# bayesiains/nflows

Measured on AMD Instinct MI355X. Metric: log_prob samples/sec (dim=64, K=8, 32-layer RQ-NSF) + max |fwd∘inv − x|, higher is better.
Workload: dtype f32 (inputs, outputs, spline arithmetic, accumulation; conditioner GEMMs: every fp32 operand carried as 3 f16 pieces = 33 significand bits, i.e. at the reference's own fp32 operand width, 5 cross products per multiply-add -- 3 on the f16 MFMA, the 2 at the 2^-22 level from the pieces' high bytes on

## Files before the change

### nflows_amd/csrc/f16x3_gemm.hpp

```cpp
#pragma once

#include "bf16x3_gemm.hpp"

namespace nfa {

typedef _Float16 f16x8 __attribute__((ext_vector_type(8)));
typedef int i32x8 __attribute__((ext_vector_type(8)));

namespace k8x {

constexpr int kScaleA = 119, kScaleB = 127;

#ifdef NFA_ABL_NO_MFMA
#define NFA_K8X_F16(a, b, c) (c)
#define NFA_K8X_BF8(a, b, c) (c)
#else
#define NFA_K8X_F16(a, b, c) __builtin_amdgcn_mfma_f32_32x32x16_f16(a, b, c, 0, 0, 0)
#define NFA_K8X_BF8(a, b, c) __builtin_amdgcn_mfma_scale_f32_32x32x64_f8f6f4(a, b, c, 1, 1, 0, kScaleA, 0, kScaleB)
#endif

struct Pieces {
    uvec4 h, l, r;
};

#define NFA_K8X_ASM asm volatile

__device__ __forceinline__ void split3_scaled(float v0, float v1, float scale, unsigned& hi, unsigned& lo, unsigned& rr) {
#if defined(NFA_K8X_NO_ASM)
    typedef _Float16 h2 __attribute__((ext_vector_type(2)));
    const float x0 = v0 * scale, x1 = v1 * scale;
    const h2 h = {(_Float16)x0, (_Float16)x1};
    const float t0 = x0 - (float)h[0], t1 = x1 - (float)h[1];
    const h2 l = {(_Float16)t0, (_Float16)t1};
    const h2 r = {(_Float16)((t0 - (float)l[0]) * 256.0f), (_Float16)((t1 - (float)l[1]) * 256.0f)};
    hi = __builtin_bit_cast(unsigned, h);
    lo = __builtin_bit_cast(unsigned, l);
    rr = __builtin_bit_cast(unsigned, r);
#else
    unsigned h, l, r;
    float t0, t1;
    NFA_K8X_ASM(
        "v_fma_mixlo_f16 %0, %5, %7, 0 op_sel_hi:[0,0,0]\n\t"
        "v_fma_mixhi_f16 %0, %6, %7, 0 op_sel_hi:[0,0,0]\n\t"
        "v_fma_mix_f32 %3, %5, %7, -%0 op_sel_hi:[0,0,1]\n\t"
        "v_fma_mix_f32 %4, %6, %7, -%0 op_sel:[0,0,1] op_sel_hi:[0,0,1]\n\t"
        "v_fma_mixlo_f16 %1, %3, 1.0, 0 op_sel_hi:[0,0,0]\n\t"
        "v_fma_mixhi_f16 %1, %4, 1.0, 0 op_sel_hi:[0,0,0]\n\t"
        "v_fma_mix_f32 %3, %3, 1.0, -%1 op_sel_hi:[0,0,1]\n\t"
        "v_fma_mix_f32 %4, %4, 1.0, -%1 op_sel:[0,0,1] op_sel_hi:[0,0,1]\n\t"
        "v_fma_mixlo_f16 %2, %3, %8, 0 op_sel_hi:[0,0,0]\n\t"
        "v_fma_mixhi_f16 %2, %4, %8, 0 op_sel_hi:[0,0,0]"
        : "=&v"(h), "=&v"(l), "=&v"(r), "=&v"(t0), "=&v"(t1)
        : "v"(v0), "v"(v1), "v"(scale), "s"(256.0f));
    hi = h;
    lo = l;
    rr = r;
#endif
}

__device__ __forceinline__ void pieces_fma2(unsigned h, unsigned l, unsigned r, float mul, float& acc0, float& acc1) {
    float t0, t1;
#if defined(NFA_K8X_NO_ASM)
    typedef _Float16 h2 __attribute__((ext_vector_type(2)));
    const h2 hh = __builtin_bit_cast(h2, h), ll = __builtin_bit_cast(h2, l), rr = __builtin_bit_cast(h2, r);
    t0 = ((float)hh[0] + (float)ll[0]) + (float)rr[0] * 0.00390625f;
    t1 = ((float)hh[1] + (float)ll[1]) + (float)rr[1] * 0.00390625f;
#else
    NFA_K8X_ASM(
        "v_fma_mix_f32 %0, %2, 1.0, %3 op_sel_hi:[1,0,1]\n\t"
        "v_fma_mix_f32 %1, %2, 1.0, %3 op_sel:[1,0,1] op_sel_hi:[1,0,1]\n\t"
        "v_fma_mix_f32 %0, %4, %5, %0 op_sel_hi:[1,0,0]\n\t"
        "v_fma_mix_f32 %1, %4, %5, %1 op_sel:[1,0,0] op_sel_hi:[1,0,0]"
        : "=&v"(t0), "=&v"(t1)
        : "v"(h), "v"(l), "v"(r), "s"(0.00390625f));
#endif
    acc0 = __builtin_fmaf(t0, mul, acc0);
    acc1 = __builtin_fmaf(t1, mul, acc1);
}

__device__ __forceinline__ void relu_pieces(Pieces& p) {
#pragma unroll
    for (int i = 0; i < 4; ++i) {
        unsigned keep;
        asm volatile("v_pk_min_i16 %0, %1, 0\n\t"
            "v_pk_add_i16 %0, %0, %2\n\t"
            "v_pk_ashrrev_i16 %0, %3, %0\n\t"
            "v_not_b32 %0, %0"
            : "=&v"(keep)
            : "v"(p.h[i]), "s"(0x03FF03FFu), "s"(0x000F000Fu));
        p.h[i] &= keep;
        p.l[i] &= keep;
        p.r[i] &= keep;
    }
}

__device__ __forceinline__ i32x8 bf8_operand(const Pieces& p0, const Pieces& p1) {
    constexpr unsigned kHigh = 0x07050301u;
    i32x8 b;
    b[0] = (int)__builtin_amdgcn_perm(p0.r[1], p0.r[0], kHigh);
    b[1] = (int)__builtin_amdgcn_perm(p0.r[3], p0.r[2], kHigh);
    b[2] = (int)__builtin_amdgcn_perm(p0.h[1], p0.h[0], kHigh);
    b[3] = (int)__builtin_amdgcn_perm(p0.h[3], p0.h[2], kHigh);
    b[4] = (int)__builtin_amdgcn_perm(p1.r[1], p1.r[0], kHigh);
    b[5] = (int)__builtin_amdgcn_perm(p1.r[3], p1.r[2], kHigh);
    b[6] = (int)__builtin_amdgcn_perm(p1.h[1], p1.h[0], kHigh);
    b[7] = (int)__builtin_amdgcn_perm(p1.h[3], p1.h[2], kHigh);
    return b;
}

template <bool RELU>
__device__ __forceinline__ void tile_to_pieces(const f32x16& a, float scale, Pieces& p0, Pieces& p1) {
    asm volatile("s_nop 7\n\ts_nop 3" : : "v"(a));
#pragma unroll
    for (int q2 = 0; q2 < 8; ++q2) {
        float v0 = a[q2 * 2], v1 = a[q2 * 2 + 1];
        if (RELU) {
            v0 = v0 < 0.0f ? 0.0f : v0;
            v1 = v1 < 0.0f ? 0.0f : v1;
        }
        unsigned h, l, r;
        split3_scaled(v0, v1, scale, h, l, r);
        if (q2 < 4) {
            p0.h[q2] = h;
            p0.l[q2] = l;
            p0.r[q2] = r;
        } else {
            p1.h[q2 - 4] = h;
            p1.l[q2 - 4] = l;
            p1.r[q2 - 4] = r;
        }
    }
}

__device__ __forceinline__ void add_pieces(f32x16& a, int q0, const Pieces& p, float mul) {
#pragma unroll
    for (int j2 = 0; j2 < 4; ++j2) {
        float a0 = a[q0 + 2 * j2], a1 = a[q0 + 2 * j2 + 1];
        pieces_fma2(p.h[j2], p.l[j2], p.r[j2], mul, a0, a1);
        a[q0 + 2 * j2] = a0;
        a[q0 + 2 * j2 + 1] = a1;
    }
}

__device__ __forceinline__ i32x8 join_x(vec4f lo, vec4f hi) {
    const uvec4 a = __builtin_bit_cast(uvec4, lo), b = __builtin_bit_cast(uvec4, hi);
    return i32x8{(int)a[0], (int)a[1], (int)a[2], (int)a[3], (int)b[0], (int)b[1], (int)b[2], (int)b[3]};
}

struct Lead {
    vec4f h0, l0, h1, l1;
};
__device__ __forceinline__ Lead read_lead(const vec4f* stage) {
    return Lead{stage[0 * 64], stage[1 * 64], stage[2 * 64], stage[3 * 64]};
}

#define NFA_K8X_FENCE() __builtin_amdgcn_sched_barrier(0)

template <bool LAST>
__device__ __forceinline__ void stage_kmajor(f32x16& acc0, f32x16& acc1, const Pieces& b0, const Pieces& b1, const i32x8& bx,
                                             WeightStream& sm, int lane, Lead& lead) {
    stream_request(sm);
    const vec4f* cur = sm.ring + sm.slot * kStageVec4 + lane;
    const f16x8 bh0 = __builtin_bit_cast(f16x8, b0.h), bl0 = __builtin_bit_cast(f16x8, b0.l);
    const f16x8 bh1 = __builtin_bit_cast(f16x8, b1.h), bl1 = __builtin_bit_cast(f16x8, b1.l);
    const vec4f x0l = cur[4 * 64], x0h = cur[5 * 64];
    const vec4f h0 = cur[6 * 64], l0 = cur[7 * 64], h1 = cur[8 * 64], l1 = cur[9 * 64], x1l = cur[10 * 64], x1h = cur[11 * 64];
    NFA_K8X_FENCE();
    {
        const f16x8 ah0 = __builtin_bit_cast(f16x8, lead.h0), al0 = __builtin_bit_cast(f16x8, lead.l0);
        const f16x8 ah1 = __builtin_bit_cast(f16x8, lead.h1), al1 = __builtin_bit_cast(f16x8, lead.l1);
        acc0 = NFA_K8X_F16(ah0, bl0, acc0);
        acc0 = NFA_K8X_F16(al0, bh0, acc0);
        acc0 = NFA_K8X_F16(ah0, bh0, acc0);
        acc0 = NFA_K8X_F16(ah1, bl1, acc0);
        acc0 = NFA_K8X_F16(al1, bh1, acc0);
        acc0 = NFA_K8X_F16(ah1, bh1, acc0);
        acc0 = NFA_K8X_BF8(join_x(x0l, x0h), bx, acc0);
    }
    const f16x8 ah0 = __builtin_bit_cast(f16x8, h0), al0 = __builtin_bit_cast(f16x8, l0);
    const f16x8 ah1 = __builtin_bit_cast(f16x8, h1), al1 = __builtin_bit_cast(f16x8, l1);
    const i32x8 ax = join_x(x1l, x1h);
    acc1 = NFA_K8X_F16(ah0, bl0, acc1);
    acc1 = NFA_K8X_F16(al0, bh0, acc1);
    acc1 = NFA_K8X_F16(ah0, bh0, acc1);
    NFA_K8X_FENCE();
    stream_advance(sm);
    if constexpr (!LAST) lead = read_lead(sm.ring + sm.slot * kStageVec4 + lane);
    NFA_K8X_FENCE();
    acc1 = NFA_K8X_F16(ah1, bl1, acc1);
    acc1 = NFA_K8X_F16(al1, bh1, acc1);
    acc1 = NFA_K8X_F16(ah1, bh1, acc1);
    acc1 = NFA_K8X_BF8(ax, bx, acc1);
}

template <bool RELU, int NKS>
__device__ __forceinline__ void gemm_kmajor(f32x16 (&acc)[4], const Pieces (&p)[8], WeightStream& sm, int lane) {
    static_assert(NKS % 2 == 0, "pairs of k-steps");
    Lead lead = read_lead(sm.ring + sm.slot * kStageVec4 + lane);
#pragma unroll
    for (int pr = 0; pr < NKS / 2; ++pr) {
        Pieces b0 = p[2 * pr], b1 = p[2 * pr + 1];
        if (RELU) {
            relu_pieces(b0);
            relu_pieces(b1);
        }
        const i32x8 bx = bf8_operand(b0, b1);
        stage_kmajor<false>(acc[0], acc[1], b0, b1, bx, sm, lane, lead);
        if (pr + 1 < NKS / 2) stage_kmajor<false>(acc[2], acc[3], b0, b1, bx, sm, lane, lead);
        else stage_kmajor<true>(acc[2], acc[3], b0, b1, bx, sm, lane, lead);
    }
}

}
}
```

### nflows_amd/csrc/rqs_resnet_f16x3_kernel.hpp

```cpp
#pragma once

#include "f16x3_gemm.hpp"
#include "rqs_resnet_f16_kernel.hpp"

#include <hip/hip_ext.h>
#include <stdlib.h>

namespace nfa {
namespace k8x {

struct Args {
    const float* x;
    const vec4f* w;
    const float* bias;
    const float* scales;
    const int32_t* tables;
    float* out;
    float* lad;
    int32_t* redo;
    int32_t* status;
    int64_t batch;
    int D, dt, di, num_blocks, num_layers, num_stages, bias_per_layer, accumulate;
    RqsDev sp;
    int normal, skip_out;
    float log_z, act_scale;
    int Ds;
    float* dbg_logits;
};

typedef __attribute__((address_space(3))) float lds_f32;

using nfa::load_bias_tile;

__device__ __forceinline__ void load_bias_tile(f32x16& acc, const lds_f32* bias_tile_half) {
    typedef __attribute__((address_space(3))) const vec4f lds_vec4f;
    lds_vec4f* bp = reinterpret_cast<lds_vec4f*>(bias_tile_half);
#pragma unroll
    for (int q4 = 0; q4 < 4; ++q4) {
        const vec4f b = bp[q4];
        acc[q4 * 4 + 0] = b.x;
        acc[q4 * 4 + 1] = b.y;
        acc[q4 * 4 + 2] = b.z;
        acc[q4 * 4 + 3] = b.w;
    }
}

template <int N>
__device__ __forceinline__ void uniform_load(const float* p, float (&v)[N]) {
    static_assert(N == 2 || N == 4, "one or two pairs");
    uint64_t v01, v23 = 0;
    if constexpr (N == 2)
        asm volatile("s_load_dwordx2 %0, %1, 0x0\n\ts_waitcnt lgkmcnt(0)" : "=&s"(v01) : "s"(p) : "memory");
    else
        asm volatile("s_load_dwordx2 %0, %2, 0x0\n\ts_load_dwordx2 %1, %2, 0x8\n\ts_waitcnt lgkmcnt(0)"
                     : "=&s"(v01), "=&s"(v23) : "s"(p) : "memory");
    v[0] = __builtin_bit_cast(float, (unsigned)v01);
    v[1] = __builtin_bit_cast(float, (unsigned)(v01 >> 32));
    if constexpr (N == 4) {
        v[2] = __builtin_bit_cast(float, (unsigned)v23);
        v[3] = __builtin_bit_cast(float, (unsigned)(v23 >> 32));
    }
}

struct NoWeave {
    template <int U0, int U1>
    __device__ __forceinline__ void span() {}
};
template <int UNIT, class Steps>
struct UnitWeave {
    Steps &fa, &fb;
    const RqsDev& sp;
    template <int U0, int U1>
    __device__ __forceinline__ void span() {
        constexpr int N = k8h::spline_unit_slices<UNIT, Steps>();
        k8h::spline_unit_range<UNIT, (U0 * N) / 32, (U1 * N) / 32>(fa, fb, sp);
    }
};
template <int MASK, class Steps>
struct SeqWeave {
    Steps& f;
    const RqsDev& sp;
    template <int U0, int U1>
    __device__ __forceinline__ void span() {
        constexpr int N = k8h::spline_seq_count<MASK, Steps>();
        k8h::spline_seq_range<MASK, (U0 * N) / 32, (U1 * N) / 32>(f, sp);
    }
};

#define NFA_K8X_PUMP_F16(U, A_, B_)                                         \
    acc = NFA_K8X_F16(A_, B_, acc);                                         \
    __builtin_amdgcn_sched_barrier(0);                                      \
    w.template span<(U), (U) + 1>();                                        \
    __builtin_amdgcn_sched_barrier(0)
#define NFA_K8X_PUMP_BF8(U, A_, B_)                                         \
    acc = NFA_K8X_BF8(A_, B_, acc);                                         \
    __builtin_amdgcn_sched_barrier(0);                                      \
    w.template span<(U), (U) + 2>();                                        \
    __builtin_amdgcn_sched_barrier(0)

template <int HS, class W>
__device__ __forceinline__ void stage_pumped(f32x16& acc, const Pieces (&p)[8], const i32x8 (&bx)[4], WeightStream& sm, int lane,
                                             Lead& lead, W& w) {
    stream_request(sm);
    const vec4f* cur = sm.ring + sm.slot * kStageVec4 + lane;
    vec4f xa = cur[8 * 64], xb = cur[9 * 64];
    vec4f fh0 = lead.h0, fl0 = lead.l0, fh1 = lead.h1, fl1 = lead.l1;
    {
        const Pieces& b0 = p[HS * 4 + 0];
        const Pieces& b1 = p[HS * 4 + 1];
        const f16x8 bh0 = __builtin_bit_cast(f16x8, b0.h), bl0 = __builtin_bit_cast(f16x8, b0.l);
        const f16x8 bh1 = __builtin_bit_cast(f16x8, b1.h), bl1 = __builtin_bit_cast(f16x8, b1.l);
        const f16x8 ah0 = __builtin_bit_cast(f16x8, fh0), al0 = __builtin_bit_cast(f16x8, fl0);
        const f16x8 ah1 = __builtin_bit_cast(f16x8, fh1), al1 = __builtin_bit_cast(f16x8, fl1);
        const i32x8 ax = join_x(xa, xb);
        NFA_K8X_PUMP_F16(HS * 16 + 0, ah0, bl0);
        NFA_K8X_PUMP_F16(HS * 16 + 1, al0, bh0);
        NFA_K8X_PUMP_F16(HS * 16 + 2, ah0, bh0);
        fh0 = cur[4 * 64];
        fl0 = cur[5 * 64];
        NFA_K8X_PUMP_F16(HS * 16 + 3, ah1, bl1);
        NFA_K8X_PUMP_F16(HS * 16 + 4, al1, bh1);
        NFA_K8X_PUMP_F16(HS * 16 + 5, ah1, bh1);
        fh1 = cur[6 * 64];
        fl1 = cur[7 * 64];
        NFA_K8X_PUMP_BF8(HS * 16 + 6, ax, bx[HS * 2 + 0]);
        xa = cur[10 * 64];
        xb = cur[11 * 64];
    }
    {
        const Pieces& b0 = p[HS * 4 + 2];
        const Pieces& b1 = p[HS * 4 + 3];
        const f16x8 bh0 = __builtin_bit_cast(f16x8, b0.h), bl0 = __builtin_bit_cast(f16x8, b0.l);
        const f16x8 bh1 = __builtin_bit_cast(f16x8, b1.h), bl1 = __builtin_bit_cast(f16x8, b1.l);
        const f16x8 ah0 = __builtin_bit_cast(f16x8, fh0), al0 = __builtin_bit_cast(f16x8, fl0);
        const f16x8 ah1 = __builtin_bit_cast(f16x8, fh1), al1 = __builtin_bit_cast(f16x8, fl1);
        const i32x8 ax = join_x(xa, xb);
        NFA_K8X_PUMP_F16(HS * 16 + 8, ah0, bl0);
        NFA_K8X_PUMP_F16(HS * 16 + 9, al0, bh0);
        NFA_K8X_PUMP_F16(HS * 16 + 10, ah0, bh0);
        NFA_K8X_PUMP_F16(HS * 16 + 11, ah1, bl1);
        NFA_K8X_PUMP_F16(HS * 16 + 12, al1, bh1);
        NFA_K8X_PUMP_F16(HS * 16 + 13, ah1, bh1);
        stream_advance(sm);
        lead = read_lead(sm.ring + sm.slot * kStageVec4 + lane);
        __builtin_amdgcn_sched_barrier(0);
        NFA_K8X_PUMP_BF8(HS * 16 + 14, ax, bx[HS * 2 + 1]);
    }
}
#undef NFA_K8X_PUMP_F16
#undef NFA_K8X_PUMP_BF8

template <class W>
__device__ __forceinline__ void gemm_tile_pumped(f32x16& acc, const Pieces (&p)[8], const i32x8 (&bx)[4], WeightStream& sm, int lane,
                                                 Lead& lead, W&& w) {
    stage_pumped<0>(acc, p, bx, sm, lane, lead, w);
    stage_pumped<1>(acc, p, bx, sm, lane, lead, w);
}

template <int TI, int T, int KB, class Steps, class BiasPtr>
__device__ __forceinline__ void any_group_tiles(f32x16& acc, Steps& f, BiasPtr gb, const Pieces (&p)[8], const i32x8 (&bx)[4],
                                                WeightStream& sm, int lane, Lead& lead, const RqsDev& sp) {
    if constexpr (TI < T) {
        constexpr int kMask = k8h::any_tile_mask(KB, TI);
        load_bias_tile(acc, gb + TI * 32);
        if constexpr (kMask != 0) gemm_tile_pumped(acc, p, bx, sm, lane, lead, SeqWeave<kMask, Steps>{f, sp});
        else gemm_tile_pumped(acc, p, bx, sm, lane, lead, NoWeave{});
        k8h::take_chunk<TI, KB>(f, acc);
        any_group_tiles<TI + 1, T, KB, Steps, BiasPtr>(acc, f, gb, p, bx, sm, lane, lead, sp);
    }
}

__device__ __forceinline__ bool not_finite(float v) { return !(__builtin_fabsf(v) < INFINITY); }

template <bool INVERSE, int INIT_KS, bool DBG = false, int KB = 8>
__global__ void __launch_bounds__(kBlock, 2) rqs_resnet_f16x3_kernel(const Args a) {
    static_assert(!DBG || KB == 8, "the diagnostic instances: 8 bins");
    constexpr int kFinalRows = KB == 8 ? 24 : 16 * ((3 * KB - 1 + 15) / 16);
    constexpr int NW = kBlock / kWave;
    extern __shared__ __attribute__((aligned(16))) float lds_dyn[];
    __shared__ int s_tab[2][kTabLayer];
    __shared__ int s_final[128];
    __shared__ int s_bad[NW];
    const int tid = threadIdx.x, lane = tid & 63, wave = __builtin_amdgcn_readfirstlane(tid >> 6);
    const int D = a.D, dt = a.dt;
    int my_status = 0;
    auto checked = [&](int v, bool used) {
        my_status |= (used && (v < 0 || v >= D)) ? NFA_STATUS_BAD_INDEX : 0;
        return v < 0 ? 0 : (v >= D ? D - 1 : v);
    };
    const int te = tid & (kTabLayer - 1);
    s_tab[0][te] = checked(a.tables[te], te < kTabTr ? te < a.di : te - kTabTr < dt);
    s_final[te] = checked(a.tables[a.num_layers * kTabLayer + te], te < D);

    WeightStream sm;
    sm.w = a.w;
    sm.ring = reinterpret_cast<vec4f*>(lds_dyn);
    sm.slot = 1;
    sm.fetch = 0;
    sm.num_stages = a.num_stages * a.num_layers;
    sm.tid = tid;
    stream_request(sm);
    sm.slot = 2;
    stream_request(sm);
    sm.slot = 0;
    asm volatile("s_waitcnt vmcnt(0)" ::: "memory");
    __syncthreads();

    lds_f32* s_row = (lds_f32*)lds_dyn + kRing * kStageVec4 * 4 + wave * D * kRowPad;
    lds_f32* s_fbias = (lds_f32*)lds_dyn + kRing * kStageVec4 * 4 + NW * D * kRowPad;
    const int groups = dt >> 2;
    const int64_t num_quads = a.batch >> 7;
    const int gemms = 2 + 2 * a.num_blocks;
    const float S = a.act_scale;
    int tb = 0;

    for (int64_t quad = blockIdx.x; quad < num_quads; quad += gridDim.x) {
        const int64_t row0 = (quad << 7) + (wave << 5);
        int lane_here = lane, di = a.di;
        asm volatile("" : "+v"(lane_here), "+s"(di));
        const int half = lane_here >> 5, r = lane_here & 31;
        {
            const vec4f* xv = reinterpret_cast<const vec4f*>(a.x + row0 * D);
            const int nvec = D * 8;
            for (int e0 = lane; e0 < nvec; e0 += kWave * 4) {
                vec4f v[4];
#pragma unroll
                for (int u = 0; u < 4; ++u) {
                    const int e = e0 + u * kWave;
                    v[u] = xv[e < nvec ? e : 0];
                }
#pragma unroll
                for (int u = 0; u < 4; ++u) {
                    const int e = e0 + u * kWave;
                    if (e < nvec) {
                        const int rr = (e * 4) / D, c0 = e * 4 - rr * D;
                        s_row[(c0 + 0) * kRowPad + rr] = v[u].x;
                        s_row[(c0 + 1) * kRowPad + rr] = v[u].y;
                        s_row[(c0 + 2) * kRowPad + rr] = v[u].z;
                        s_row[(c0 + 3) * kRowPad + rr] = v[u].w;
                    }
                }
            }
        }
        __builtin_amdgcn_fence(__ATOMIC_RELEASE, "wavefront");
        __builtin_amdgcn_fence(__ATOMIC_ACQUIRE, "wavefront");

        float lad_acc = 0.0f;
        int quad_status = 0;
        for (int layer = 0; layer < a.num_layers; ++layer) {
            if ((layer + (blockIdx.x >= (gridDim.x >> 1) ? 1 : 0)) & 1) __builtin_amdgcn_s_setprio(1);
            else __builtin_amdgcn_s_setprio(0);
            const int* tab = s_tab[tb];
            {
                unsigned all = ~0u;
                asm volatile("" : "+s"(all));
                const int te_l = (int)__builtin_amdgcn_mbcnt_hi(all, __builtin_amdgcn_mbcnt_lo(all, 0u)) + ((wave & 1) << 6);
                const int nl = layer + 1 < a.num_layers ? layer + 1 : 0;
                s_tab[tb ^ 1][te_l] = checked(a.tables[nl * kTabLayer + te_l], te_l < kTabTr ? te_l < a.di : te_l - kTabTr < dt);
            }
            const float* bias = a.bias + (size_t)layer * a.bias_per_layer + half * 16;
            const float* sc = a.scales + (size_t)layer * gemms * 2;
            Pieces p[8];

#pragma unroll
            for (int ks = 0; ks < INIT_KS; ++ks) {
#pragma unroll
                for (int j2 = 0; j2 < 4; ++j2) {
                    const int i0 = ks * 16 + half * 8 + j2 * 2;
                    float v0 = s_row[tab[kTabId + i0] * kRowPad + r], v1 = s_row[tab[kTabId + i0 + 1] * kRowPad + r];
                    v0 = i0 < di ? v0 : 0.0f;
                    v1 = i0 + 1 < di ? v1 : 0.0f;
                    unsigned hi, lo, rr;
                    split3_scaled(v0, v1, S, hi, lo, rr);
                    p[ks].h[j2] = hi;
                    p[ks].l[j2] = lo;
                    p[ks].r[j2] = rr;
                }
            }

            {
                f32x16 h[4];
#pragma unroll
                for (int t = 0; t < 4; ++t) load_bias_tile(h[t], bias + t * 32);
                gemm_kmajor<false, INIT_KS>(h, p, sm, lane);
                float s0[2];
                uniform_load(sc, s0);
                const float inv_t = s0[0];
#pragma unroll
                for (int t = 0; t < 4; ++t) tile_to_pieces<false>(h[t], inv_t, p[2 * t], p[2 * t + 1]);
            }
            bias += 128;
            sc += 2;
            {
                const float* fbias = a.bias + (size_t)layer * a.bias_per_layer + 128 + 256 * a.num_blocks;
                for (int i = tid; i < dt * kFinalRows; i += kBlock) s_fbias[i] = fbias[i];
                if (a.num_blocks == 0) __syncthreads();
            }

            for (int blk = 0; blk < a.num_blocks; ++blk) {
                f32x16 v[4];
                Pieces q[8];
                float sb[4];
                {
                    f32x16 u[4];
#pragma unroll
                    for (int t = 0; t < 4; ++t) load_bias_tile(u[t], bias + t * 32);
                    gemm_kmajor<true, 8>(u, p, sm, lane);
                    uniform_load(sc, sb);
                    const float t1 = sb[3];
#pragma unroll
                    for (int t = 0; t < 4; ++t) {
                        load_bias_tile(v[t], bias + 128 + t * 32);
                        add_pieces(v[t], 0, p[2 * t], t1);
                        add_pieces(v[t], 8, p[2 * t + 1], t1);
                    }
                    const float inv_t = sb[0];
#pragma unroll
                    for (int t = 0; t < 4; ++t) tile_to_pieces<true>(u[t], inv_t, q[2 * t], q[2 * t + 1]);
                }
                const float inv_t1 = sb[2];
                gemm_kmajor<false, 8>(v, q, sm, lane);
#pragma unroll
                for (int t = 0; t < 4; ++t) tile_to_pieces<false>(v[t], inv_t1, p[2 * t], p[2 * t + 1]);
                bias += 256;
                sc += 4;
            }

            if constexpr (KB == 8) {
                using Steps = FusedSteps<INVERSE, 8>;
                Steps fa{}, fb{};
                float sf[2];
                uniform_load(sc, sf);
                const float kappa = sf[0];
                fa.kappa = fb.kappa = kappa;
                fa.kl2e = fb.kl2e = 1.44269502162933349609375f * kappa;
                fa.tail_s = fb.tail_s = a.sp.tail_logit * sf[1];
                lds_f32* slot_b = s_row;
                const lds_f32* fbias = s_fbias + half * 16;
                i32x8 bx[4];
#pragma unroll
                for (int j = 0; j < 4; ++j) bx[j] = bf8_operand(p[2 * j], p[2 * j + 1]);
                Lead lead = read_lead(sm.ring + sm.slot * kStageVec4 + lane);
                f32x16 acc[3];
                auto commit = [&](Steps& f, lds_f32* slot) {
                    *slot = f.y;
                    lad_acc += f.lad;
                    quad_status |= f.status;
                };
                [[maybe_unused]] auto store_logits = [&](const f32x16& t, int tile) {
                    if constexpr (DBG) {
                        if (layer == a.num_layers - 1) {
                            float* dst = a.dbg_logits + (size_t)(row0 + r) * (dt * kFinalRows) + tile * 32 + half * 16;
#pragma unroll
                            for (int q_ = 0; q_ < 16; ++q_) dst[q_] = t[q_] * kappa;
                            asm volatile("s_waitcnt vmcnt(0)" ::: "memory");
                        }
                    }
                };
                UnitWeave<k8h::kUnitNumA, Steps> w0{fa, fb, a.sp};
                UnitWeave<k8h::kUnitFinishA, Steps> w1{fa, fb, a.sp};
                UnitWeave<k8h::kUnitFinishB, Steps> w2{fa, fb, a.sp};
                for (int g = 0; g < groups; ++g) {
                    lds_f32* slot0 = s_row + tab[kTabTr + g * 4 + half * 2] * kRowPad + r;
                    lds_f32* slot1 = s_row + tab[kTabTr + g * 4 + half * 2 + 1] * kRowPad + r;
                    load_bias_tile(acc[0], fbias + (g * 3 + 0) * 32);
                    if (g > 0) {
                        gemm_tile_pumped(acc[0], p, bx, sm, lane, lead, w2);
                        commit(fb, slot_b);
                    } else {
                        gemm_tile_pumped(acc[0], p, bx, sm, lane, lead, NoWeave{});
                    }
                    store_logits(acc[0], g * 3 + 0);
                    fa.x = *slot0;
#pragma unroll
                    for (int j = 0; j < 8; ++j) {
                        fa.ew[j] = acc[0][j];
                        fa.eh[j] = acc[0][8 + j];
                    }
                    load_bias_tile(acc[1], fbias + (g * 3 + 1) * 32);
                    gemm_tile_pumped(acc[1], p, bx, sm, lane, lead, w0);
                    store_logits(acc[1], g * 3 + 1);
                    fb.x = *slot1;
#pragma unroll
                    for (int j = 0; j < 8; ++j) {
                        if (j < 7) fa.sd[j] = acc[1][j];
                        fb.ew[j] = acc[1][8 + j];
                    }
                    load_bias_tile(acc[2], fbias + (g * 3 + 2) * 32);
                    gemm_tile_pumped(acc[2], p, bx, sm, lane, lead, w1);
                    store_logits(acc[2], g * 3 + 2);
                    commit(fa, slot0);
#pragma unroll
                    for (int j = 0; j < 8; ++j) {
                        fb.eh[j] = acc[2][j];
                        if (j < 7) fb.sd[j] = acc[2][8 + j];
                    }
                    slot_b = slot1;
                }
                k8h::spline_unit_range<k8h::kUnitFinishB, 0, k8h::spline_unit_slices<k8h::kUnitFinishB, Steps>()>(fa, fb, a.sp);
                commit(fb, slot_b);
            }
            else {
                constexpr int T = kFinalRows / 16;
                static_assert(T >= 1 && T <= 6, "2 .. 32 bins");
                using Steps = FusedSteps<INVERSE, KB>;
                constexpr int kRest = k8h::any_rest_mask(KB);
                Steps f{};
                float sf[2];
                uniform_load(sc, sf);
                const float kappa = sf[0];
                f.kappa = kappa;
                f.kl2e = 1.44269502162933349609375f * kappa;
                f.tail_s = a.sp.tail_logit * sf[1];
                const lds_f32* fbias = s_fbias + half * 16;
                i32x8 bx[4];
#pragma unroll
                for (int j = 0; j < 4; ++j) bx[j] = bf8_operand(p[2 * j], p[2 * j + 1]);
                Lead lead = read_lead(sm.ring + sm.slot * kStageVec4 + lane);
                const int groups_any = dt >> 1;
                f32x16 acc;
                lds_f32* slot = s_row + tab[kTabTr + half] * kRowPad + r;
                load_bias_tile(acc, fbias);
                gemm_tile_pumped(acc, p, bx, sm, lane, lead, NoWeave{});
                for (int g = 0; g < groups_any; ++g) {
                    const lds_f32* gb = fbias + g * T * 32;
                    f.x = *slot;
                    k8h::take_chunk<0, KB>(f, acc);
                    any_group_tiles<1, T, KB, Steps>(acc, f, gb, p, bx, sm, lane, lead, a.sp);
                    if (g + 1 < groups_any) {
                        lds_f32* next_slot = s_row + tab[kTabTr + (g + 1) * 2 + half] * kRowPad + r;
                        load_bias_tile(acc, gb + T * 32);
                        gemm_tile_pumped(acc, p, bx, sm, lane, lead, SeqWeave<kRest, Steps>{f, a.sp});
                        *slot = f.y;
                        slot = next_slot;
                    } else {
                        k8h::spline_seq_range<kRest, 0, k8h::spline_seq_count<kRest, Steps>()>(f, a.sp);
                        *slot = f.y;
                    }
                    lad_acc += f.lad;
                    quad_status |= f.status;
                }
            }
            tb ^= 1;
            __builtin_amdgcn_fence(__ATOMIC_RELEASE, "wavefront");
            __builtin_amdgcn_fence(__ATOMIC_ACQUIRE, "wavefront");
        }

        lad_acc += __shfl_xor(lad_acc, 32, kWave);
        const float sumsq = tile_row_sumsq((const float*)s_row, a.Ds, half, r);
        const bool bad = not_finite(lad_acc) || not_finite(sumsq);
        const bool wave_bad = __builtin_amdgcn_ballot_w64(bad) != 0;
        if (lane == 0) s_bad[wave] = wave_bad ? 1 : 0;
        asm volatile("s_waitcnt vmcnt(0)" ::: "memory");
        __syncthreads();
        int any_bad = 0;
#pragma unroll
        for (int w_ = 0; w_ < NW; ++w_) any_bad |= s_bad[w_];
        if (!any_bad) {
            if (!a.skip_out) {
                vec4f* ov = reinterpret_cast<vec4f*>(a.out + row0 * D);
                const int nvec = D * 8;
                for (int e = lane; e < nvec; e += kWave) {
                    const int rr = (e * 4) / D, c0 = e * 4 - rr * D;
                    vec4f v;
                    v.x = s_row[s_final[c0 + 0] * kRowPad + rr];
                    v.y = s_row[s_final[c0 + 1] * kRowPad + rr];
                    v.z = s_row[s_final[c0 + 2] * kRowPad + rr];
                    v.w = s_row[s_final[c0 + 3] * kRowPad + rr];
                    ov[e] = v;
                }
            }
            if (half == 0) {
                float* dst = a.lad + row0 + r;
                float v = a.accumulate ? *dst + lad_acc : lad_acc;
                if (a.normal) v = (-0.5f * sumsq - a.log_z) + v;
                *dst = v;
            }
            my_status |= quad_status;
        }
        if (tid == 0) a.redo[quad] = any_bad ? 1 : 0;
        asm volatile("s_waitcnt vmcnt(0)" ::: "memory");
        __syncthreads();
    }
    asm volatile("s_waitcnt vmcnt(0)" ::: "memory");
    if (my_status && a.status) atomicOr(a.status, my_status);
}

}
}


namespace nfa {
namespace k8x {
typedef void (*KernelFn)(const Args);
KernelFn bins_kernel_a(int K, bool inverse, int init_ks);
KernelFn bins_kernel_b(int K, bool inverse, int init_ks);
}
}
```

Baseline: 26.07 million.

## Keep residual stream in fp32 and split into f16 pieces lazily inside the GEMM

```diff
diff --git a/nflows_amd/csrc/f16x3_gemm.hpp b/nflows_amd/csrc/f16x3_gemm.hpp
--- a/nflows_amd/csrc/f16x3_gemm.hpp
+++ b/nflows_amd/csrc/f16x3_gemm.hpp
@@ -19,15 +19,42 @@
 #define NFA_K8X_BF8(a, b, c) __builtin_amdgcn_mfma_scale_f32_32x32x64_f8f6f4(a, b, c, 1, 1, 0, kScaleA, 0, kScaleB)
 #endif
 
+__device__ __forceinline__ void request_stage(WeightStream& sm) {
+    const int dst_slot = sm.slot >= 1 ? sm.slot - 1 : kRing - 1;
+    const char* stage = reinterpret_cast<const char*>(sm.w) + (size_t)sm.fetch * (kStageVec4 * 16);
+    const __amdgpu_buffer_rsrc_t rsrc =
+        __builtin_amdgcn_make_buffer_rsrc(const_cast<char*>(stage), (short)0, kStageVec4 * 16, 0x00020000);
+    const int wave = __builtin_amdgcn_readfirstlane(sm.tid >> 6);
+    char* slot = reinterpret_cast<char*>(sm.ring) + dst_slot * (kStageVec4 * 16) + wave * (kWave * 16);
+    const unsigned lane_off = (unsigned)sm.tid * 16u;
+#pragma unroll
+    for (int i = 0; i < 3; ++i)
+        __builtin_amdgcn_raw_ptr_buffer_load_lds(rsrc, (__attribute__((address_space(3))) void*)(slot + i * kBlock * 16), 16,
+                                                 lane_off, i * kBlock * 16, 0, 0);
+    sm.fetch = (sm.fetch + 1 == sm.num_stages) ? 0 : sm.fetch + 1;
+}
+
 struct Pieces {
     uvec4 h, l, r;
 };
 
 #define NFA_K8X_ASM asm volatile
 
+#define NFA_K8X_SPLIT_REST                                                  \
+    "v_fma_mixlo_f16 %1, %3, 1.0, 0 op_sel_hi:[0,0,0]\n\t"                  \
+    "v_fma_mixhi_f16 %1, %4, 1.0, 0 op_sel_hi:[0,0,0]\n\t"                  \
+    "v_fma_mix_f32 %3, %3, 1.0, -%1 op_sel_hi:[0,0,1]\n\t"                  \
+    "v_fma_mix_f32 %4, %4, 1.0, -%1 op_sel:[0,0,1] op_sel_hi:[0,0,1]\n\t"   \
+    "v_fma_mixlo_f16 %2, %3, %8, 0 op_sel_hi:[0,0,0]\n\t"                   \
+    "v_fma_mixhi_f16 %2, %4, %8, 0 op_sel_hi:[0,0,0]"
+template <bool RELU = false>
 __device__ __forceinline__ void split3_scaled(float v0, float v1, float scale, unsigned& hi, unsigned& lo, unsigned& rr) {
 #if defined(NFA_K8X_NO_ASM)
     typedef _Float16 h2 __attribute__((ext_vector_type(2)));
+    if (RELU) {
+        v0 = __builtin_isnan(v0) ? v0 : (v0 > 0.0f ? v0 : 0.0f);
+        v1 = __builtin_isnan(v1) ? v1 : (v1 > 0.0f ? v1 : 0.0f);
+    }
     const float x0 = v0 * scale, x1 = v1 * scale;
     const h2 h = {(_Float16)x0, (_Float16)x1};
     const float t0 = x0 - (float)h[0], t1 = x1 - (float)h[1];
@@ -39,60 +66,32 @@
 #else
     unsigned h, l, r;
     float t0, t1;
-    NFA_K8X_ASM(
-        "v_fma_mixlo_f16 %0, %5, %7, 0 op_sel_hi:[0,0,0]\n\t"
-        "v_fma_mixhi_f16 %0, %6, %7, 0 op_sel_hi:[0,0,0]\n\t"
-        "v_fma_mix_f32 %3, %5, %7, -%0 op_sel_hi:[0,0,1]\n\t"
-        "v_fma_mix_f32 %4, %6, %7, -%0 op_sel:[0,0,1] op_sel_hi:[0,0,1]\n\t"
-        "v_fma_mixlo_f16 %1, %3, 1.0, 0 op_sel_hi:[0,0,0]\n\t"
-        "v_fma_mixhi_f16 %1, %4, 1.0, 0 op_sel_hi:[0,0,0]\n\t"
-        "v_fma_mix_f32 %3, %3, 1.0, -%1 op_sel_hi:[0,0,1]\n\t"
-        "v_fma_mix_f32 %4, %4, 1.0, -%1 op_sel:[0,0,1] op_sel_hi:[0,0,1]\n\t"
-        "v_fma_mixlo_f16 %2, %3, %8, 0 op_sel_hi:[0,0,0]\n\t"
-        "v_fma_mixhi_f16 %2, %4, %8, 0 op_sel_hi:[0,0,0]"
-        : "=&v"(h), "=&v"(l), "=&v"(r), "=&v"(t0), "=&v"(t1)
-        : "v"(v0), "v"(v1), "v"(scale), "s"(256.0f));
+    if constexpr (RELU)
+        NFA_K8X_ASM(
+            "v_maximum3_f32 %3, %5, 0, 0\n\t"
+            "v_maximum3_f32 %4, %6, 0, 0\n\t"
+            "v_fma_mixlo_f16 %0, %3, %7, 0 op_sel_hi:[0,0,0]\n\t"
+            "v_fma_mixhi_f16 %0, %4, %7, 0 op_sel_hi:[0,0,0]\n\t"
+            "v_fma_mix_f32 %3, %3, %7, -%0 op_sel_hi:[0,0,1]\n\t"
+            "v_fma_mix_f32 %4, %4, %7, -%0 op_sel:[0,0,1] op_sel_hi:[0,0,1]\n\t"
+            NFA_K8X_SPLIT_REST
+            : "=&v"(h), "=&v"(l), "=&v"(r), "=&v"(t0), "=&v"(t1)
+            : "v"(v0), "v"(v1), "v"(scale), "s"(256.0f));
+    else
+        NFA_K8X_ASM(
+            "v_fma_mixlo_f16 %0, %5, %7, 0 op_sel_hi:[0,0,0]\n\t"
+            "v_fma_mixhi_f16 %0, %6, %7, 0 op_sel_hi:[0,0,0]\n\t"
+            "v_fma_mix_f32 %3, %5, %7, -%0 op_sel_hi:[0,0,1]\n\t"
+            "v_fma_mix_f32 %4, %6, %7, -%0 op_sel:[0,0,1] op_sel_hi:[0,0,1]\n\t"
+            NFA_K8X_SPLIT_REST
+            : "=&v"(h), "=&v"(l), "=&v"(r), "=&v"(t0), "=&v"(t1)
+            : "v"(v0), "v"(v1), "v"(scale), "s"(256.0f));
     hi = h;
     lo = l;
     rr = r;
 #endif
 }
-
-__device__ __forceinline__ void pieces_fma2(unsigned h, unsigned l, unsigned r, float mul, float& acc0, float& acc1) {
-    float t0, t1;
-#if defined(NFA_K8X_NO_ASM)
-    typedef _Float16 h2 __attribute__((ext_vector_type(2)));
-    const h2 hh = __builtin_bit_cast(h2, h), ll = __builtin_bit_cast(h2, l), rr = __builtin_bit_cast(h2, r);
-    t0 = ((float)hh[0] + (float)ll[0]) + (float)rr[0] * 0.00390625f;
-    t1 = ((float)hh[1] + (float)ll[1]) + (float)rr[1] * 0.00390625f;
-#else
-    NFA_K8X_ASM(
-        "v_fma_mix_f32 %0, %2, 1.0, %3 op_sel_hi:[1,0,1]\n\t"
-        "v_fma_mix_f32 %1, %2, 1.0, %3 op_sel:[1,0,1] op_sel_hi:[1,0,1]\n\t"
-        "v_fma_mix_f32 %0, %4, %5, %0 op_sel_hi:[1,0,0]\n\t"
-        "v_fma_mix_f32 %1, %4, %5, %1 op_sel:[1,0,0] op_sel_hi:[1,0,0]"
-        : "=&v"(t0), "=&v"(t1)
-        : "v"(h), "v"(l), "v"(r), "s"(0.00390625f));
-#endif
-    acc0 = __builtin_fmaf(t0, mul, acc0);
-    acc1 = __builtin_fmaf(t1, mul, acc1);
-}
-
-__device__ __forceinline__ void relu_pieces(Pieces& p) {
-#pragma unroll
-    for (int i = 0; i < 4; ++i) {
-        unsigned keep;
-        asm volatile("v_pk_min_i16 %0, %1, 0\n\t"
-            "v_pk_add_i16 %0, %0, %2\n\t"
-            "v_pk_ashrrev_i16 %0, %3, %0\n\t"
-            "v_not_b32 %0, %0"
-            : "=&v"(keep)
-            : "v"(p.h[i]), "s"(0x03FF03FFu), "s"(0x000F000Fu));
-        p.h[i] &= keep;
-        p.l[i] &= keep;
-        p.r[i] &= keep;
-    }
-}
+#undef NFA_K8X_SPLIT_REST
 
 __device__ __forceinline__ i32x8 bf8_operand(const Pieces& p0, const Pieces& p1) {
     constexpr unsigned kHigh = 0x07050301u;
@@ -108,18 +107,13 @@
     return b;
 }
 
-template <bool RELU>
+template <bool RELU, bool WB = true>
 __device__ __forceinline__ void tile_to_pieces(const f32x16& a, float scale, Pieces& p0, Pieces& p1) {
-    asm volatile("s_nop 7\n\ts_nop 3" : : "v"(a));
+    if constexpr (WB) asm volatile("s_nop 7\n\ts_nop 3" : : "v"(a));
 #pragma unroll
     for (int q2 = 0; q2 < 8; ++q2) {
-        float v0 = a[q2 * 2], v1 = a[q2 * 2 + 1];
-        if (RELU) {
-            v0 = v0 < 0.0f ? 0.0f : v0;
-            v1 = v1 < 0.0f ? 0.0f : v1;
-        }
         unsigned h, l, r;
-        split3_scaled(v0, v1, scale, h, l, r);
+        split3_scaled<RELU>(a[q2 * 2], a[q2 * 2 + 1], scale, h, l, r);
         if (q2 < 4) {
             p0.h[q2] = h;
             p0.l[q2] = l;
@@ -132,16 +126,6 @@
     }
 }
 
-__device__ __forceinline__ void add_pieces(f32x16& a, int q0, const Pieces& p, float mul) {
-#pragma unroll
-    for (int j2 = 0; j2 < 4; ++j2) {
-        float a0 = a[q0 + 2 * j2], a1 = a[q0 + 2 * j2 + 1];
-        pieces_fma2(p.h[j2], p.l[j2], p.r[j2], mul, a0, a1);
-        a[q0 + 2 * j2] = a0;
-        a[q0 + 2 * j2 + 1] = a1;
-    }
-}
-
 __device__ __forceinline__ i32x8 join_x(vec4f lo, vec4f hi) {
     const uvec4 a = __builtin_bit_cast(uvec4, lo), b = __builtin_bit_cast(uvec4, hi);
     return i32x8{(int)a[0], (int)a[1], (int)a[2], (int)a[3], (int)b[0], (int)b[1], (int)b[2], (int)b[3]};
@@ -159,7 +143,7 @@
 template <bool LAST>
 __device__ __forceinline__ void stage_kmajor(f32x16& acc0, f32x16& acc1, const Pieces& b0, const Pieces& b1, const i32x8& bx,
                                              WeightStream& sm, int lane, Lead& lead) {
-    stream_request(sm);
+    request_stage(sm);
     const vec4f* cur = sm.ring + sm.slot * kStageVec4 + lane;
     const f16x8 bh0 = __builtin_bit_cast(f16x8, b0.h), bl0 = __builtin_bit_cast(f16x8, b0.l);
     const f16x8 bh1 = __builtin_bit_cast(f16x8, b1.h), bl1 = __builtin_bit_cast(f16x8, b1.l);
@@ -193,17 +177,14 @@
     acc1 = NFA_K8X_BF8(ax, bx, acc1);
 }
 
-template <bool RELU, int NKS>
-__device__ __forceinline__ void gemm_kmajor(f32x16 (&acc)[4], const Pieces (&p)[8], WeightStream& sm, int lane) {
+template <int NKS, class PairFn>
+__device__ __forceinline__ void gemm_kmajor_pairs(f32x16 (&acc)[4], WeightStream& sm, int lane, PairFn&& pair) {
     static_assert(NKS % 2 == 0, "pairs of k-steps");
     Lead lead = read_lead(sm.ring + sm.slot * kStageVec4 + lane);
 #pragma unroll
     for (int pr = 0; pr < NKS / 2; ++pr) {
-        Pieces b0 = p[2 * pr], b1 = p[2 * pr + 1];
-        if (RELU) {
-            relu_pieces(b0);
-            relu_pieces(b1);
-        }
+        Pieces b0, b1;
+        pair(pr, b0, b1);
         const i32x8 bx = bf8_operand(b0, b1);
         stage_kmajor<false>(acc[0], acc[1], b0, b1, bx, sm, lane, lead);
         if (pr + 1 < NKS / 2) stage_kmajor<false>(acc[2], acc[3], b0, b1, bx, sm, lane, lead);
@@ -211,5 +192,21 @@
     }
 }
 
-}
-}
+template <int NKS>
+__device__ __forceinline__ void gemm_kmajor(f32x16 (&acc)[4], const Pieces (&p)[8], WeightStream& sm, int lane) {
+    gemm_kmajor_pairs<NKS>(acc, sm, lane, [&](int pr, Pieces& b0, Pieces& b1) {
+        b0 = p[2 * pr];
+        b1 = p[2 * pr + 1];
+    });
+}
+
+__device__ __forceinline__ void gemm_kmajor_relu(f32x16 (&acc)[4], const f32x16 (&src)[4], float scale, WeightStream& sm,
+                                                 int lane) {
+    gemm_kmajor_pairs<8>(acc, sm, lane, [&](int pr, Pieces& b0, Pieces& b1) {
+        if (pr == 0) tile_to_pieces<true, true>(src[pr], scale, b0, b1);
+        else tile_to_pieces<true, false>(src[pr], scale, b0, b1);
+    });
+}
+
+}
+}
diff --git a/nflows_amd/csrc/rqs_resnet_f16x3_kernel.hpp b/nflows_amd/csrc/rqs_resnet_f16x3_kernel.hpp
--- a/nflows_amd/csrc/rqs_resnet_f16x3_kernel.hpp
+++ b/nflows_amd/csrc/rqs_resnet_f16x3_kernel.hpp
@@ -101,7 +101,7 @@
 template <int HS, class W>
 __device__ __forceinline__ void stage_pumped(f32x16& acc, const Pieces (&p)[8], const i32x8 (&bx)[4], WeightStream& sm, int lane,
                                              Lead& lead, W& w) {
-    stream_request(sm);
+    request_stage(sm);
     const vec4f* cur = sm.ring + sm.slot * kStageVec4 + lane;
     vec4f xa = cur[8 * 64], xb = cur[9 * 64];
     vec4f fh0 = lead.h0, fl0 = lead.l0, fh1 = lead.h1, fl1 = lead.l1;
@@ -199,9 +199,9 @@
     sm.fetch = 0;
     sm.num_stages = a.num_stages * a.num_layers;
     sm.tid = tid;
-    stream_request(sm);
+    request_stage(sm);
     sm.slot = 2;
-    stream_request(sm);
+    request_stage(sm);
     sm.slot = 0;
     asm volatile("s_waitcnt vmcnt(0)" ::: "memory");
     __syncthreads();
@@ -278,16 +278,15 @@
                 }
             }
 
+            f32x16 h[4];
+            float hs;
             {
-                f32x16 h[4];
 #pragma unroll
                 for (int t = 0; t < 4; ++t) load_bias_tile(h[t], bias + t * 32);
-                gemm_kmajor<false, INIT_KS>(h, p, sm, lane);
+                gemm_kmajor<INIT_KS>(h, p, sm, lane);
                 float s0[2];
                 uniform_load(sc, s0);
-                const float inv_t = s0[0];
-#pragma unroll
-                for (int t = 0; t < 4; ++t) tile_to_pieces<false>(h[t], inv_t, p[2 * t], p[2 * t + 1]);
+                hs = s0[0];
             }
             bias += 128;
             sc += 2;
@@ -298,33 +297,28 @@
             }
 
             for (int blk = 0; blk < a.num_blocks; ++blk) {
-                f32x16 v[4];
-                Pieces q[8];
                 float sb[4];
-                {
-                    f32x16 u[4];
-#pragma unroll
-                    for (int t = 0; t < 4; ++t) load_bias_tile(u[t], bias + t * 32);
-                    gemm_kmajor<true, 8>(u, p, sm, lane);
-                    uniform_load(sc, sb);
-                    const float t1 = sb[3];
-#pragma unroll
-                    for (int t = 0; t < 4; ++t) {
-                        load_bias_tile(v[t], bias + 128 + t * 32);
-                        add_pieces(v[t], 0, p[2 * t], t1);
-                        add_pieces(v[t], 8, p[2 * t + 1], t1);
-                    }
-                    const float inv_t = sb[0];
-#pragma unroll
-                    for (int t = 0; t < 4; ++t) tile_to_pieces<true>(u[t], inv_t, q[2 * t], q[2 * t + 1]);
-                }
-                const float inv_t1 = sb[2];
-                gemm_kmajor<false, 8>(v, q, sm, lane);
-#pragma unroll
-                for (int t = 0; t < 4; ++t) tile_to_pieces<false>(v[t], inv_t1, p[2 * t], p[2 * t + 1]);
+                f32x16 u[4];
+#pragma unroll
+                for (int t = 0; t < 4; ++t) load_bias_tile(u[t], bias + t * 32);
+                gemm_kmajor_relu(u, h, hs, sm, lane);
+                uniform_load(sc, sb);
+                const float skip = hs * sb[3];
+#pragma unroll
+                for (int t = 0; t < 4; ++t) {
+                    f32x16 b1;
+                    load_bias_tile(b1, bias + 128 + t * 32);
+#pragma unroll
+                    for (int q_ = 0; q_ < 16; ++q_) h[t][q_] = __builtin_fmaf(h[t][q_], skip, b1[q_]);
+                }
+                gemm_kmajor_relu(h, u, sb[0], sm, lane);
+                hs = sb[2];
                 bias += 256;
                 sc += 4;
             }
+
+#pragma unroll
+            for (int t = 0; t < 4; ++t) tile_to_pieces<false>(h[t], hs, p[2 * t], p[2 * t + 1]);
 
             if constexpr (KB == 8) {
                 using Steps = FusedSteps<INVERSE, 8>;
```

After: 27.42 million (median of 6 runs). 5.2% higher.
